# iosefa/obia

Hardware: AMD Instinct MI355X
Metric: Mpixel/s (SLIC+zonal feats) on 16384²×8-band; achieved HBM GB/s fraction (higher is better)
Workload: dtype f32

## Files before the change

### obia_amd/csrc/slic_sweep.hip

```cpp
#include "slic.hpp"

#include <type_traits>
#include <hip/hip_ext.h>

#include <cstdlib>

namespace obia {

#ifdef OBIA_STAMP
__device__ unsigned long long g_tl[65536 * 4 * 24];
#define STAMP_DECL unsigned long long st_t = clock64(), st_t0 = st_t, st_r0 = __builtin_amdgcn_s_memrealtime(), st_acc[12] = {0, 0, 0, 0, 0, 0, 0, 0, 0, 0, 0, 0}, st_cnt[6] = {0, 0, 0, 0, 0, 0};
#define STAMP_COUNT(i, v) st_cnt[i] += (v);
#define STAMP(i) { const unsigned long long st_n = clock64(); st_acc[i] += st_n - st_t; st_t = st_n; }
#ifndef OBIA_STAMP_KIND
#define OBIA_STAMP_KIND 0
#endif
#define STAMP_FLUSH if (accumulate && (LEAN ? 1 : 0) == OBIA_STAMP_KIND && (threadIdx.x & 63) == 0 && gtile < 65536) { unsigned long long *st_o = g_tl + ((size_t)gtile * 4 + (threadIdx.x >> 6)) * 24; for (int st_i = 0; st_i < 12; ++st_i) st_o[st_i] = st_acc[st_i]; st_o[12] = st_t0; st_o[13] = clock64(); st_o[14] = st_r0; st_o[15] = __builtin_amdgcn_s_memrealtime(); for (int st_i = 0; st_i < 6; ++st_i) st_o[16 + st_i] = st_cnt[st_i]; }
#else
#define STAMP_DECL
#define STAMP(i)
#define STAMP_COUNT(i, v)
#define STAMP_FLUSH
#endif

// ... 692 lines not shown
            key = (key == mn) ? 0xffffffffu : key;
            float clb = 0.0f;
            if (COLLB) clb = __uint_as_float(__builtin_amdgcn_readlane(__float_as_uint(clbv), sl));
            const float4 *__restrict__ crec = reinterpret_cast<const float4 *>(cent + (size_t)kk * RS);
            const float4 h0 = crec[0], h1 = crec[1];
            const unsigned mn_next = wave_umin(key);
            const float cy = h0.x, cx = h0.y;
            const int y0 = __float_as_int(h0.z), y1 = __float_as_int(h0.w);
            const int x0 = __float_as_int(h1.x), x1 = __float_as_int(h1.y);
            const float mdc = SLICZERO ? h1.w : 1.0f;
            mn = mn_next;
            STAMP(8)
            const float tx = cx - fx;
            const float dx2 = tx * tx;
            int yb_v = yb_i;
            asm volatile("" : "+v"(yb_v));
            const float fyb = (float)yb_v;
            v2f dv2[PPT / 2];
#pragma unroll
            for (int p = 0; p < PPT / 2; ++p) {
                const v2f tyv = splat(cy) - (splat(fyb) + (v2f){(float)(2 * p), (float)(2 * p + 1)});
                const v2f dy2 = tyv * tyv;
                dv2[p] = (dy2 + splat(dx2)) * splat(w);
            }
            float dv[PPT] = {dv2[0].x, dv2[0].y, dv2[1].x, dv2[1].y};
            if (!((y0 <= fy0) && (y1 >= fy1) && (x0 <= fx0) && (x1 >= fx1))) {
                const bool inx = (x >= x0) && (x < x1);
#pragma unroll
                for (int j = 0; j < PPT; ++j)
                    dv[j] = (inx && ((unsigned)(yb_v + j - y0) < (unsigned)(y1 - y0))) ? dv[j] : INFINITY;
            }
            const bool anylive = COLLB ? (!(dv[0] + clb > BK_D(0)) || !(dv[1] + clb > BK_D(1)) || !(dv[2] + clb > BK_D(2)) || !(dv[3] + clb > BK_D(3)))
                                       : (!(dv[0] > BK_D(0)) || !(dv[1] > BK_D(1)) || !(dv[2] > BK_D(2)) || !(dv[3] > BK_D(3)));
            STAMP_COUNT(1, 1)
            STAMP(9)
            if (!firstv && !__ballot(anylive)) continue;
            STAMP_COUNT(2, 1)
            STAMP_COUNT(3, 2)
            {
                float col[LEAN ? 1 : CP];
                if (!IGNORE_COLOR) {
#pragma unroll
                    for (int q = 0; q < (NCH + 3) / 4; ++q) {
                        const float4 t = crec[2 + q];
                        col[4 * q] = t.x; col[4 * q + 1] = t.y; col[4 * q + 2] = t.z; col[4 * q + 3] = t.w;
                    }
                }
                v2f d0 = (v2f){dv[0], dv[1]}, d1 = (v2f){dv[2], dv[3]};
                if (!IGNORE_COLOR) {
                    v2f t0 = f2[0][0] - splat(col[0]), t1 = f2[0][1] - splat(col[0]);
                    v2f dc0 = t0 * t0, dc1 = t1 * t1;
#pragma unroll
                    for (int ch = 1; ch < (LEAN ? 1 : NCH); ++ch) {
                        t0 = f2[LEAN ? 0 : ch][0] - splat(col[LEAN ? 0 : ch]);
                        t1 = f2[LEAN ? 0 : ch][1] - splat(col[LEAN ? 0 : ch]);
                        dc0 += t0 * t0;
                        dc1 += t1 * t1;
                    }
                    d0 += SLICZERO ? dc0 / splat(mdc) : dc0;
                    d1 += SLICZERO ? dc1 / splat(mdc) : dc1;
                }
                const float dd[PPT] = {d0.x, d0.y, d1.x, d1.y};
                if (firstv) {
#pragma unroll
                    for (int j = 0; j < PPT; ++j) {
                        const unsigned long long nk = ((unsigned long long)__float_as_uint(dd[j]) << 32) | (unsigned long long)c;
                        bk[j] = (dd[j] < INFINITY) ? nk : bk[j];
                    }
                    firstv = false;
                } else
#pragma unroll
                for (int j = 0; j < PPT; ++j) {
                    const unsigned long long nk = ((unsigned long long)__float_as_uint(dd[j]) << 32) | (unsigned long long)c;
                    bk[j] = (nk < bk[j]) ? nk : bk[j];
                }
            }
            mybest = fmaxf(fmaxf(BK_D(0), BK_D(1)), fmaxf(BK_D(2), BK_D(3)));
            STAMP(10)
        }
        STAMP(3)

        int pk[PPT];
        int32_t *lbase = labels + (P.pix_off + (long long)fy0 * P.W + fx0);
        bool orphan = false;
        bool valid[PPT];
#pragma unroll
        for (int j = 0; j < PPT; ++j) {
            const bool inimg = (yb_i + j < P.H) && (x < P.W);
            valid[j] = inimg && (((mbw >> (8 * j)) & 0xffu) != 0u);
            const bool assigned = valid[j] && ((unsigned)(bk[j] >> 32) < INF_BITS);
            pk[j] = assigned ? (int)(unsigned)bk[j] : -1;
            orphan |= valid[j] && !assigned;
        }
        if (store_labels) {
#pragma unroll
            for (int j = 0; j < PPT; ++j) {
                const bool inimg = (yb_i + j < P.H) && (x < P.W);
                const int kk = s_k[(unsigned)bk[j]];
                if (inimg && !(valid[j] && pk[j] < 0))
                    __builtin_nontemporal_store(pk[j] >= 0 ? kk - P.cent_off + start_label : start_label - 1,
                                                lbase + (lrow_i + (unsigned)j * (unsigned)P.W));
            }
        }
        if (__ballot(orphan)) {
            if (orphan_needs_repeat(store_labels, sweep_id) && lane_i == 0) *orphan_flag = 1;
#pragma unroll
            for (int j = 0; j < PPT; ++j)
                if (valid[j] && ((unsigned)(bk[j] >> 32) >= INF_BITS)) {
                    const int ry = yb_i + j - ty0, rx = x - tx0;
                    atomicOr(&s_orph[ry * (SWEEP_TW / 32) + (rx >> 5)], 1u << (rx & 31));
                    s_uncacheable = 1;
                }
        }
        STAMP(4)

        if (accumulate) {
        if (FOLD_LAYERS > 0) s_tkey[wv][0][lane_i] = -1;
        if (FOLD_LAYERS > 1) s_tkey[wv][1][lane_i] = -1;
        {
            const unsigned xrel = (unsigned)(x - tx0);
            int rkey = -1, nruns = 0;
            unsigned pw = 0;
            int rf[LEAN ? 1 : CP];
#pragma unroll
            for (int ch = 0; ch < (LEAN ? 1 : CP); ++ch) rf[ch] = 0;
            auto close_run = [&]() {
                if (rkey < 0) return;
                if (nruns < FOLD_LAYERS) {
                    s_tkey[wv][nruns][lane_i] = rkey;
                    s_tf[wv][nruns][NF - 1][lane_i] = (int)pw;
                    if (!LEAN && accum_color) {
#pragma unroll
                        for (int ch = 0; ch < CP; ++ch) s_tf[wv][nruns][LEAN ? 0 : ch][lane_i] = rf[LEAN ? 0 : ch];
                    }
                } else {
                    atomicAdd(&s_acc[rkey][PWI], (unsigned long long)(pw & 0xffu) | ((unsigned long long)((pw >> 8) & 0xfffu) << 16) |
                                                     ((unsigned long long)(pw >> 20) << 40));
                    if (!LEAN && accum_color) {
#pragma unroll
                        for (int ch = 0; ch < CP; ++ch) atomicAdd(&s_acc[rkey][LEAN ? 0 : ch], (unsigned long long)(long long)rf[LEAN ? 0 : ch]);
                    }
                }
                ++nruns;
            };
            auto merge_strip = [&](auto pre_tag) {
                constexpr bool PRE = decltype(pre_tag)::value;
#pragma unroll
                for (int j = 0; j < PPT; ++j) {
                    if (pk[j] != rkey) {
                        close_run();
                        rkey = pk[j]; pw = 0;
#pragma unroll
                        for (int ch = 0; ch < (LEAN ? 1 : CP); ++ch) rf[ch] = 0;
                    }
                    if (pk[j] >= 0) {
                        pw += 1u | ((unsigned)(yb_i + j - ty0) << 8) | (xrel << 20);
                        if (!LEAN && accum_color) {
#pragma unroll
                            for (int ch = 0; ch < NCH; ++ch) {
                                const float fv = (j & 1) ? f2[LEAN ? 0 : ch][j >> 1].y : f2[LEAN ? 0 : ch][j >> 1].x;
                                rf[LEAN ? 0 : ch] += PRE ? (int)fv : to_fixed32(fv, fs);
                            }
                        }
                    }
                }
                close_run();
            };
            if (fs == 1.0f) merge_strip(std::true_type{});
            else merge_strip(std::false_type{});
        }
        }
        STAMP(5)
        {
            const bool has_next = (bxi + 1 < SWEEP_TW / FB) && (fx0 + FB < P.W);
            fetch(has_next ? fx0 + FB : fx0, yb_i, lane_i, has_next);
        }
        if (!accumulate || FOLD_LAYERS == 0) continue;
        wave_lds_sync();
        if (!LEAN && accum_color) {
#pragma unroll
            for (int pass = 0; pass < NPASS; ++pass) {
                const int fld = 8 * pass + (lane_i & 7), g = lane_i >> 3;
                if (fld < CP) {
#pragma unroll
                    for (int layer = 0; layer < FOLD_LAYERS; ++layer) {
                        int cur = -1;
                        long long sum = 0;
                        int tkv[8], vv[8];
#pragma unroll
                        for (int i = 0; i < 8; ++i) { tkv[i] = s_tkey[wv][layer][8 * g + i]; vv[i] = s_tf[wv][layer][LEAN ? 0 : fld][8 * g + i]; }
#pragma unroll
                        for (int i = 0; i < 8; ++i) {
                            const int tk = tkv[i];
                            const int v = vv[i];
                            if (tk != cur) {
                                if (cur >= 0) atomicAdd(&s_acc[cur][LEAN ? 0 : fld], (unsigned long long)sum);
                                cur = tk; sum = 0;
                            }
                            sum += (long long)v;
                        }
                        if (cur >= 0) atomicAdd(&s_acc[cur][LEAN ? 0 : fld], (unsigned long long)sum);
                    }
                }
            }
        }
        if (lane_i < 8 * FOLD_LAYERS) {
            const int layer = lane_i >> 3, g = lane_i & 7;
            int cur = -1;
            unsigned sum = 0;
            auto emit = [&]() {
                atomicAdd(&s_acc[cur][PWI], (unsigned long long)(sum & 0xffu) | ((unsigned long long)((sum >> 8) & 0xfffu) << 16) |
                                                ((unsigned long long)(sum >> 20) << 40));
            };
            int tkv[8];
            unsigned vv[8];
#pragma unroll
            for (int i = 0; i < 8; ++i) { tkv[i] = s_tkey[wv][layer][8 * g + i]; vv[i] = (unsigned)s_tf[wv][layer][NF - 1][8 * g + i]; }
#pragma unroll
            for (int i = 0; i < 8; ++i) {
                const int tk = tkv[i];
                const unsigned v = vv[i];
                if (tk != cur) {
                    if (cur >= 0) emit();
                    cur = tk; sum = 0;
                }
                sum += v;
            }
            if (cur >= 0) emit();
        }
        wave_lds_sync();
        STAMP(6)
    }
#undef BK_D
    if (!accumulate) { STAMP_FLUSH return; }
    __syncthreads();
    const int tid_e = wv * 64 + lane_now();
    if (s_uncacheable && store_labels == 2) {
        for (int i = tid_e; i < SWEEP_TH * SWEEP_TW; i += NT) {
            if (!((s_orph[i >> 5] >> (i & 31)) & 1u)) continue;
            const int y = ty0 + i / SWEEP_TW, x = tx0 + i % SWEEP_TW;
            const long long pix = P.pix_off + (long long)y * P.W + x;
            const int prev = labels[pix];
            if (prev < start_label) continue;
            float one[CP];
#pragma unroll
            for (int ch = 0; ch < CP; ++ch) one[ch] = (accum_color && ch < nch_rt) ? feat_at(feat, P, CP, y, x, ch) : 0.0f;
            global_accumulate<CP>(acc, RQ, prev - start_label + P.cent_off, (unsigned)y, (unsigned)x, one, fs);
        }
    }
    const bool keep = FIXPT && !s_uncacheable;
    int *ck = keep ? cache_k + (size_t)tile_id * (MAXC + 1) : nullptr;
    unsigned long long *cq = keep ? cache_q + (size_t)tile_id * MAXC * GQ : nullptr;
    constexpr int QLO = (LEAN && !FIXPT) ? CP : 0, QN = GQ - QLO;
    for (int i = tid_e; i < nc * QN; i += NT) {
        const int slot = i / QN, q = QLO + (i - slot * QN);
        const unsigned long long pw = s_acc[slot][PWI];
        const unsigned long long n = pw & 0xffffull;
        if (FIXPT && keep && q == QLO) ck[1 + slot] = n ? s_k[slot] : -1;
        if (n == 0ull) continue;
        const int k = s_k[slot];
        unsigned long long v;
        if (q < CP) { if (!FIXPT && !accum_color) continue; v = accum_color ? s_acc[slot][LEAN ? 0 : q] : 0ull; }
        else if (q == CP) v = n;
        else if (q == CP + 1) v = ((pw >> 16) & 0xffffffull) + n * (unsigned long long)ty0;
        else v = (pw >> 40) + n * (unsigned long long)tx0;
        if (FIXPT && keep) cq[(size_t)slot * GQ + q] = v;
        if (FIXPT && q < CP && !accum_color) continue;
        atomicAdd(&acc[(size_t)k * RQ + q], v);
    }
    if (keep && tid_e == 0) { ck[0] = nc; tile_lp[tile_id] = sweep_id; }
    STAMP(7)
    STAMP_FLUSH
}

#define OBIA_ASSIGN_PARAMS                                                                                             \
    const SlicProblem *__restrict__ probs, const float *__restrict__ feat, const uint8_t *__restrict__ mask,             \
        const unsigned *__restrict__ mask4, const float *__restrict__ cent, const int *__restrict__ head,                                                    \
        int32_t *__restrict__ labels, unsigned long long *__restrict__ acc, int RQ, int accumulate, int store_labels,     \
        int start_label, float fs, const int *__restrict__ bin_stamp, int *__restrict__ tile_lp,                    \
        int *__restrict__ cache_k, unsigned long long *__restrict__ cache_q, int sweep_id, int use_cache,                 \
        unsigned long long *__restrict__ px_counter, const int *__restrict__ tile_prob, int total_tiles_all,              \
        int *__restrict__ orphan_flag, int tiles_per_prob, const float *__restrict__ fbox, int tile_base, int nch_arg,     \
        int *__restrict__ tl_k, unsigned *__restrict__ tl_fp, int *__restrict__ tl_meta, const int *__restrict__ tl_req
#define OBIA_ASSIGN_ARGS                                                                                               \
    probs, feat, mask, mask4, cent, head, labels, acc, RQ, accumulate, store_labels, start_label, fs, bin_stamp, tile_lp, \
        cache_k, cache_q, sweep_id, use_cache, px_counter, tile_prob, total_tiles_all, orphan_flag, tiles_per_prob, fbox, tile_base, nch_arg, \
        tl_k, tl_fp, tl_meta, tl_req

template <int CP, bool MASKED, bool IGNORE_COLOR, bool FIXPT, bool SLICZERO, int NCH = CP>
__global__ __launch_bounds__(NT) __attribute__((amdgpu_waves_per_eu(ASSIGN_WAVES, ASSIGN_WAVES))) void slic_assign_kernel(OBIA_ASSIGN_PARAMS) {
    slic_assign_body<CP, MASKED, IGNORE_COLOR, FIXPT, SLICZERO, false, false, NCH>(OBIA_ASSIGN_ARGS);
}

template <int CP, bool MASKED, int NCH = CP>
__global__ __launch_bounds__(NT) __attribute__((amdgpu_waves_per_eu(6, 6))) void slic_assign_collb_kernel(OBIA_ASSIGN_PARAMS) {
    slic_assign_body<CP, MASKED, false, false, false, false, true, NCH>(OBIA_ASSIGN_ARGS);
}

template <int CP, bool MASKED, bool FIXPT>
__global__ __launch_bounds__(NT) __attribute__((amdgpu_waves_per_eu(LEAN_WAVES, LEAN_WAVES))) void slic_prepass_kernel(OBIA_ASSIGN_PARAMS) {
    slic_assign_body<CP, MASKED, true, FIXPT, false, true, false>(OBIA_ASSIGN_ARGS);
}

#ifdef OBIA_STAMP
extern "C" void obia_debug_timeline(unsigned long long *out, int nwaves) {
    (void)hipMemcpyFromSymbol(out, HIP_SYMBOL(g_tl), sizeof(unsigned long long) * 24 * (size_t)nwaves);
}
#endif

template <int CP, bool MASKED>
__global__ __launch_bounds__(256) void slic_maxdist_kernel(const SlicProblem *__restrict__ probs, const float *__restrict__ feat,
                                                           const uint8_t *__restrict__ mask, const int32_t *__restrict__ labels,
                                                           float *__restrict__ cent, int start_label, int nch) {
    constexpr int RS = CENT_REC + CP;
    const SlicProblem P = probs[blockIdx.y];
    for (int y = blockIdx.x; y < P.H; y += gridDim.x)
        for (int x = threadIdx.x; x < P.W; x += 256) {
            const long long pix = P.pix_off + (long long)y * P.W + x;
            if (MASKED && mask[pix] == 0) continue;
            const int l = labels[pix];
            if (l < start_label) continue;
            const int k = l - start_label + P.cent_off;
            const float *rec = cent + (size_t)k * RS;
            float dc = 0.0f;
#pragma unroll
            for (int ch = 0; ch < CP; ++ch) {
                if (ch >= nch) break;
                const float t = feat_at(feat, P, CP, y, x, ch) - rec[CENT_REC + ch];
                dc += t * t;
            }
            unsigned *slot = reinterpret_cast<unsigned *>(cent + (size_t)k * RS + 7);
            if (__float_as_uint(dc) > __hip_atomic_load(slot, __ATOMIC_RELAXED, __HIP_MEMORY_SCOPE_AGENT)) atomicMax(slot, __float_as_uint(dc));
        }
}

struct FixedPointState {
    int *bin_stamp = nullptr, *tile_lp = nullptr, *cache_k = nullptr;
    unsigned long long *cache_q = nullptr;
};

template <int CP>
static void launch_assign(obia_ctx *ctx, SlicBatch &b, int ignore_color, int accumulate, int accum_color, int store_labels,
                          int *orphan_flag, const FixedPointState &fp, int sweep_id, int use_cache, unsigned long long *px_counter,
                          const KernelSpan &span, const int *head_cur) {
    constexpr int XGH = OBIA_XCD_GROUP;
    const int ntiles = (int)b.total_tiles_all;
    dim3 grid(8 * XGH * (unsigned)((ntiles + 8 * XGH - 1) / (8 * XGH)));
    const int RQ = acc_record_qwords(CP);
    int tpp = b.probs.empty() ? 0 : b.probs[0].tiles_x * b.probs[0].tiles_y;
    for (auto &P : b.probs) if (P.tiles_x * P.tiles_y != tpp) tpp = 0;
#define LAUNCH_K_(...)                                                                                               \
    hipExtLaunchKernelGGL(HIP_KERNEL_NAME(__VA_ARGS__), grid, dim3(NT), 0, ctx->stream, span.a, span.b, 0, b.d_probs, b.d_feat,   \
                          b.d_mask, b.d_mask4, b.d_cent, head_cur, b.d_labels, b.d_acc, RQ, accumulate, store_labels, b.start_label,      \
                          (float)b.fscale, fp.bin_stamp, fp.tile_lp, fp.cache_k, fp.cache_q, sweep_id, use_cache, px_counter,          \
                          b.d_tile_prob, ntiles, orphan_flag, tpp, b.d_fbox, 0, b.C, b.d_tl_k, b.d_tl_fp, b.d_tl_meta, b.d_tl_req)
    const int pad = CP - b.C;
#define LAUNCH_ASSIGN_(M, I, F, Z) LAUNCH_K_(slic_assign_kernel<CP, M, I, F, Z>)
#define LAUNCH_MAIN_(M)                                                                                              \
    do {                                                                                                             \
        if (pad == 1) LAUNCH_K_(slic_assign_kernel<CP, M, false, false, false, CP - 1>);                             \
        else if (pad == 2) LAUNCH_K_(slic_assign_kernel<CP, M, false, false, false, CP - 2>);                        \
        else if (pad == 3) LAUNCH_K_(slic_assign_kernel<CP, M, false, false, false, CP - 3>);                        \
        else LAUNCH_K_(slic_assign_kernel<CP, M, false, false, false>);                                              \
    } while (0)
#define LAUNCH_COLLB_(M)                                                                                             \
    do {                                                                                                             \
        if (pad == 1) LAUNCH_K_(slic_assign_collb_kernel<CP, M, CP - 1>);                                            \
        else if (pad == 2) LAUNCH_K_(slic_assign_collb_kernel<CP, M, CP - 2>);                                       \
        else if (pad == 3) LAUNCH_K_(slic_assign_collb_kernel<CP, M, CP - 3>);                                       \
        else LAUNCH_K_(slic_assign_collb_kernel<CP, M>);                                                             \
    } while (0)
#define LAUNCH_LEAN_(M, F) LAUNCH_K_(slic_prepass_kernel<CP, M, F>)
#define LAUNCH_ASSIGN(M, I)                                                                                          \
    do {                                                                                                             \
        if ((I) && !accum_color) { if (fp.bin_stamp) LAUNCH_LEAN_(M, true); else LAUNCH_LEAN_(M, false); }           \
        else if (b.slic_zero && !(I)) LAUNCH_ASSIGN_(M, false, false, true);                                         \
        else if (fp.bin_stamp) LAUNCH_ASSIGN_(M, I, true, false);                                                    \
        else if (b.col_lb && b.d_fbox && !(I)) LAUNCH_COLLB_(M);                                                     \
        else if (!(I)) LAUNCH_MAIN_(M);                                                                              \
        else LAUNCH_ASSIGN_(M, I, false, false);                                                                     \
    } while (0)
    if (b.masked) { if (ignore_color) LAUNCH_ASSIGN(true, true); else LAUNCH_ASSIGN(true, false); }
    else LAUNCH_ASSIGN(false, false);
#undef LAUNCH_ASSIGN
#undef LAUNCH_ASSIGN_
#undef LAUNCH_LEAN_
#undef LAUNCH_COLLB_
#undef LAUNCH_MAIN_
#undef LAUNCH_K_
}

__global__ __launch_bounds__(256) void mask_pack4_kernel(const SlicProblem *__restrict__ probs, const uint8_t *__restrict__ mask,
                                                         unsigned *__restrict__ mask4) {
    const SlicProblem P = probs[blockIdx.y];
    if ((long long)P.n_valid == (long long)P.H * (long long)P.W) return;
    const int nq = (P.H + 3) >> 2, W = P.W;
    const uint8_t *mb = mask + P.pix_off;
    unsigned *out = mask4 + P.m4_off;
    const bool vec = (W % 4 == 0) && (P.pix_off % 4 == 0) && (P.m4_off % 4 == 0) && (reinterpret_cast<uintptr_t>(mask) % 4 == 0) &&
                     (reinterpret_cast<uintptr_t>(mask4) % 16 == 0);
    for (int q = blockIdx.x; q < nq; q += gridDim.x) {
        if (vec) {
            for (int x4 = threadIdx.x; x4 < (W >> 2); x4 += 256) {
                unsigned r[4];
#pragma unroll
                for (int j = 0; j < 4; ++j) {
                    const int y = 4 * q + j;
                    r[j] = y < P.H ? *reinterpret_cast<const unsigned *>(mb + (long long)y * W + 4 * x4) : 0u;
                }
                uint4 o;
                unsigned *ov = &o.x;
#pragma unroll
                for (int c = 0; c < 4; ++c) {
                    unsigned w = 0u;
#pragma unroll
                    for (int j = 0; j < 4; ++j) w |= (unsigned)(((r[j] >> (8 * c)) & 0xffu) != 0u) << (8 * j);
                    ov[c] = w;
                }
                *reinterpret_cast<uint4 *>(out + (long long)q * W + 4 * x4) = o;
            }
        } else {
            for (int x = threadIdx.x; x < W; x += 256) {
                unsigned w = 0u;
#pragma unroll
                for (int j = 0; j < 4; ++j) {
                    const int y = 4 * q + j;
                    if (y < P.H) w |= (unsigned)(mb[(long long)y * W + x] != 0) << (8 * j);
                }
                out[(long long)q * W + x] = w;
            }
        }
    }
}

__global__ void fill_i32_kernel(int32_t *p, long long n, int32_t v) {
    for (long long i = (long long)blockIdx.x * blockDim.x + threadIdx.x; i < n; i += (long long)gridDim.x * blockDim.x) p[i] = v;
}

static void fill_labels(obia_ctx *ctx, SlicBatch &b) {
    const long long n = b.total_pix;
    int blocks = cdiv(n, 256 * 8);
    if (blocks > 65535) blocks = 65535;
    if (blocks < 1) blocks = 1;
    hipLaunchKernelGGL(fill_i32_kernel, dim3(blocks), dim3(256), 0, ctx->stream, b.d_labels, n, b.start_label - 1);
}

static void fold_counters(obia_ctx *ctx, const unsigned long long *h) {
    if (ctx->profiling)
        for (int i = 0; i < 256; ++i) { ctx->timing.assign_px += (double)h[i]; ctx->timing.prepass_px += (double)h[256 + i]; }
}

static int queue_sweeps(obia_ctx *ctx, SlicBatch &b, bool repeat, unsigned long long **d_px_out) {
    *d_px_out = nullptr;
    if (std::getenv("OBIA_DEBUG_SYNC"))
        for (size_t p = 0; p < b.probs.size(); ++p) {
            const SlicProblem &P = b.probs[p];
            fprintf(stderr, "[obia debug]   problem %zu: %dx%d K %d steps %d %d bins %dx%d cell_off %d cent_off %d tiles %dx%d tile_off %d n_valid %d (total_cent %d total_cells %d tiles_all %lld)\n",
                    p, P.H, P.W, P.K, P.sy, P.sx, P.ncy, P.ncx, P.cell_off, P.cent_off, P.tiles_y, P.tiles_x, P.tile_off, P.n_valid,
                    b.total_cent, b.total_cells, b.total_tiles_all);
        }
    if (b.total_tiles <= 0 || b.max_iter <= 0) { fill_labels(ctx, b); return OBIA_OK; }
    for (auto &P : b.probs)
        if (P.W >= (1 << 22)) { set_error("rasters / tile windows wider than 4194303 pixels are not supported (got %d)", P.W); return OBIA_E_UNSUPPORTED; }
    const int passes = b.masked ? 2 : 1;
    const int RQ = acc_record_qwords(b.CP);
    Arena &A = ctx->arena;
    unsigned long long *d_px = A.get<unsigned long long>(513);
    if (!d_px) return OBIA_E_NOMEM;
    int *d_orphan = reinterpret_cast<int *>(d_px + 512);
    FixedPointState fp;
    if (b.exit_on_fixed_point) {
        const size_t nt = (size_t)b.total_tiles_all;
        fp.bin_stamp = A.get<int>((size_t)b.total_cells);
        fp.tile_lp = A.get<int>(nt);
        fp.cache_k = A.get<int>(nt * (MAXC + 1));
        fp.cache_q = A.get<unsigned long long>(nt * MAXC * (size_t)(b.CP + 3));
        if (!fp.bin_stamp || !fp.tile_lp || !fp.cache_k || !fp.cache_q) return OBIA_E_NOMEM;
        OBIA_HIP_TRY(hipMemsetAsync(fp.bin_stamp, 0, sizeof(int) * (size_t)b.total_cells, ctx->stream));
        OBIA_HIP_TRY(hipMemsetAsync(fp.tile_lp, 0, sizeof(int) * nt, ctx->stream));
    }
    {
        const size_t nt = (size_t)b.total_tiles_all;
        b.d_tl_k = A.get<int>(nt * MAXC);
        b.d_tl_fp = A.get<unsigned>(nt * NT);
        b.d_tl_meta = A.get<int>(nt * 3);
        b.d_tl_req = b.d_tl_meta ? b.d_tl_meta + nt * 2 : nullptr;
        b.d_ref = A.get<float>((size_t)b.total_cent * 2);
        if (!b.d_tl_k || !b.d_tl_fp || !b.d_tl_meta || !b.d_tl_req || !b.d_ref) return OBIA_E_NOMEM;
    }
    int maxh_z = 1, kmax = 1;
    for (auto &P : b.probs) { if (P.H > maxh_z) maxh_z = P.H; if (P.K > kmax) kmax = P.K; }
    if (b.masked && b.d_mask && !b.d_mask4) {
        b.d_mask4 = A.get<unsigned>((size_t)b.total_m4);
        if (!b.d_mask4) return OBIA_E_NOMEM;
        int gq = (maxh_z + 3) / 4;
        if (gq > 16384) gq = 16384;
        hipLaunchKernelGGL(mask_pack4_kernel, dim3(gq, b.nprob), dim3(256), 0, ctx->stream, b.d_probs, b.d_mask, b.d_mask4);
    }
    if (maxh_z > 4096) maxh_z = 4096;

    const bool store_all = repeat || b.exit_on_fixed_point || b.slic_zero;
    if (store_all || passes * b.max_iter <= 1) {
        fill_labels(ctx, b);
        debug_sync(ctx, "sweeps: label fill");
    }
    if (repeat) OBIA_HIP_TRY(hipMemsetAsync(b.d_acc, 0, sizeof(unsigned long long) * (size_t)b.total_cent * RQ, ctx->stream));
    const bool prep_grouped = std::getenv("OBIA_PREP_GROUPED") != nullptr;
    OBIA_HIP_TRY(hipMemsetAsync(d_px, 0, sizeof(unsigned long long) * 513, ctx->stream));
    OBIA_HIP_TRY(hipMemsetAsync(b.d_head, 0xff, sizeof(int) * (size_t)b.total_cells, ctx->stream));
    OBIA_HIP_TRY(hipMemsetAsync(b.d_tl_meta, 0xff, sizeof(int) * 3 * (size_t)b.total_tiles_all, ctx->stream));
    debug_sync(ctx, "sweeps: memsets");
    bool first = true;
    int sweep_no = 0;
    for (int pass = 0; pass < passes; ++pass) {
        const int ignore_color = (b.masked && pass == 0) ? 1 : 0;
        const bool last_pass = (pass == passes - 1);
        if (pass > 0 && store_all) {
            fill_labels(ctx, b);
            if (fp.tile_lp) OBIA_HIP_TRY(hipMemsetAsync(fp.tile_lp, 0, sizeof(int) * (size_t)b.total_tiles_all, ctx->stream));
        }
        for (int it = 0; it < b.max_iter; ++it) {
            int *head_cur = b.d_head + (size_t)(sweep_no & 1) * b.total_cells;
            int *head_nxt = b.d_head + (size_t)((sweep_no + 1) & 1) * b.total_cells;
            ++sweep_no;
            const int zmode = (b.slic_zero && !ignore_color) ? (it == 0 ? 2 : 1) : 0;
#define LAUNCH_PREP_LANE(CPV)                                                                                         \
    hipLaunchKernelGGL(HIP_KERNEL_NAME(slic_prep_lane_kernel<CPV>), dim3(cdiv(kmax, 64), b.nprob), dim3(64), 0, ctx->stream, \
                       b.d_probs, 0, first ? 1 : 0, zmode, b.d_seed, b.d_acc, RQ, 1.0 / b.fscale, b.d_cent, head_cur, head_nxt, \
                       b.total_cells, fp.bin_stamp, sweep_no, 0, b.d_ref, b.d_tl_req)
            if (!prep_grouped) {
                switch (b.CP) {
                    case 4: LAUNCH_PREP_LANE(4); break;
                    case 8: LAUNCH_PREP_LANE(8); break;
                    case 12: LAUNCH_PREP_LANE(12); break;
                    default: LAUNCH_PREP_LANE(16); break;
                }
            } else if (RQ == 16)
                hipLaunchKernelGGL(HIP_KERNEL_NAME(slic_prep_kernel<16>), dim3(cdiv(b.total_cent * 16LL, 256)), dim3(256), 0,
                                   ctx->stream, b.d_probs, b.d_cent_prob, b.total_cent, b.CP, first ? 1 : 0, zmode, b.d_seed, b.d_acc,
                                   1.0 / b.fscale, b.d_cent, head_cur, head_nxt, b.total_cells, fp.bin_stamp, sweep_no, 0, 0, b.d_ref, b.d_tl_req);
            else
                hipLaunchKernelGGL(HIP_KERNEL_NAME(slic_prep_kernel<32>), dim3(cdiv(b.total_cent * 32LL, 256)), dim3(256), 0,
                                   ctx->stream, b.d_probs, b.d_cent_prob, b.total_cent, b.CP, first ? 1 : 0, zmode, b.d_seed, b.d_acc,
                                   1.0 / b.fscale, b.d_cent, head_cur, head_nxt, b.total_cells, fp.bin_stamp, sweep_no, 0, 0, b.d_ref, b.d_tl_req);
#undef LAUNCH_PREP_LANE
            b.d_head_cur = head_cur;
            debug_sync(ctx, "sweeps: prep");
            first = false;
            if (zmode == 1) {
                dim3 zg(maxh_z, b.nprob);
#define LAUNCH_MAXDIST(CPV)                                                                                           \
    do {                                                                                                              \
        if (b.masked) hipLaunchKernelGGL(HIP_KERNEL_NAME(slic_maxdist_kernel<CPV, true>), zg, dim3(256), 0, ctx->stream, b.d_probs, \
                                         b.d_feat, b.d_mask, b.d_labels, b.d_cent, b.start_label, b.C);            \
        else hipLaunchKernelGGL(HIP_KERNEL_NAME(slic_maxdist_kernel<CPV, false>), zg, dim3(256), 0, ctx->stream, b.d_probs, \
                                b.d_feat, b.d_mask, b.d_labels, b.d_cent, b.start_label, b.C);                     \
    } while (0)
                switch (b.CP) {
                    case 4: LAUNCH_MAXDIST(4); break;
                    case 8: LAUNCH_MAXDIST(8); break;
                    case 12: LAUNCH_MAXDIST(12); break;
                    default: LAUNCH_MAXDIST(16); break;
                }
#undef LAUNCH_MAXDIST
            }
            const bool very_last = last_pass && it == b.max_iter - 1;
            const int accumulate = very_last ? 0 : 1;
            const int accum_color = (!ignore_color || it == b.max_iter - 1) ? 1 : 0;
            const int store_labels = store_all ? 2 : (very_last ? 1 : 0);
            const int use_cache = (ignore_color && it == b.max_iter - 1) ? 0 : 1;
            {
                KernelSpan span(ctx, ignore_color ? T_PREPASS : T_ASSIGN);
                unsigned long long *pxc = ctx->profiling ? d_px + (ignore_color ? 256 : 0) : nullptr;
                if (ctx->profiling && !ignore_color && store_labels) ctx->timing.assign_store_px += (double)b.total_pix;
                switch (b.CP) {
                    case 8: launch_assign<8>(ctx, b, ignore_color, accumulate, accum_color, store_labels, d_orphan, fp, sweep_no, use_cache, pxc, span, head_cur); break;
#ifndef OBIA_ONLY_CP8
                    case 4: launch_assign<4>(ctx, b, ignore_color, accumulate, accum_color, store_labels, d_orphan, fp, sweep_no, use_cache, pxc, span, head_cur); break;
                    case 12: launch_assign<12>(ctx, b, ignore_color, accumulate, accum_color, store_labels, d_orphan, fp, sweep_no, use_cache, pxc, span, head_cur); break;
                    case 16: launch_assign<16>(ctx, b, ignore_color, accumulate, accum_color, store_labels, d_orphan, fp, sweep_no, use_cache, pxc, span, head_cur); break;
#endif
                    default: set_error("bad CP"); return OBIA_E_INVALID;
                }
            }
            debug_sync(ctx, ignore_color ? "sweeps: pre-pass sweep" : "sweeps: colour sweep");
        }
    }
    OBIA_HIP_TRY(hipGetLastError());
    *d_px_out = d_px;
    return OBIA_OK;
}

int slic_run_sweeps(obia_ctx *ctx, SlicBatch &b) {
    ctx->defer_pending = false;
    unsigned long long *d_px = nullptr;
    OBIA_TRY(queue_sweeps(ctx, b, false, &d_px));
    if (!d_px) return OBIA_OK;
    if (!ctx->defer_buf) OBIA_HIP_TRY(hipHostMalloc(reinterpret_cast<void **>(&ctx->defer_buf), sizeof(unsigned long long) * 513, hipHostMallocDefault));
    OBIA_HIP_TRY(hipMemcpyAsync(ctx->defer_buf, d_px, sizeof(unsigned long long) * 513, hipMemcpyDeviceToHost, ctx->stream));
    ctx->defer_pending = true;
    return OBIA_OK;
}

int slic_sweeps_settle(obia_ctx *ctx, bool *repeat) {
    *repeat = false;
    if (!ctx->defer_pending) return OBIA_OK;
    ctx->defer_pending = false;
    const unsigned long long *h = ctx->defer_buf;
    if ((h[512] & 0xffffffffull) != 0ull) { *repeat = true; return OBIA_OK; }
    fold_counters(ctx, h);
    return OBIA_OK;
}

int slic_rerun_storing(obia_ctx *ctx, SlicBatch &b) {
    ctx->timing.batch_repeats += 1;
    unsigned long long *d_px = nullptr;
    OBIA_TRY(queue_sweeps(ctx, b, true, &d_px));
    if (!d_px) return OBIA_OK;
    unsigned long long h[513];
    OBIA_TRY(read_back(ctx, h, d_px, sizeof(h)));
    fold_counters(ctx, h);
    return OBIA_OK;
}

}
```

Before: 6489.

## Add run-based spatial-only prepass kernel exploiting distance convexity along rows

Adds a specialized kernel for the spatial-only (ignore-colour) prepass sweeps. Each 16-pixel row run is assigned by evaluating candidate centroids only at its endpoints (plus a split point), and falls back to per-pixel queues when margins are too small. Candidates are pruned per 16x16 block with lower and upper distance bounds, and counts and coordinate sums are accumulated as packed LDS atomics. This replaces per-pixel distance evaluation in masked prepass sweeps that do not store labels, at the cost of added code complexity and floating-point tie-margin heuristics.

```diff
diff --git a/obia_amd/csrc/slic_spatial.hip b/obia_amd/csrc/slic_spatial.hip
--- /dev/null
+++ b/obia_amd/csrc/slic_spatial.hip
@@ -0,0 +1,284 @@
+
+#ifdef OBIA_RUN_STATS
+__device__ unsigned long long g_run_stats[16];
+#define RS_DECL unsigned long long rs_t = clock64(); unsigned rs_c[8] = {0, 0, 0, 0, 0, 0, 0, 0};
+#define RS_COUNT(i, v) rs_c[i] += (unsigned)(v);
+#define RS_TICK(i) { const unsigned long long rs_n = clock64(); if ((threadIdx.x & 63) == 0) atomicAdd(&g_run_stats[i], rs_n - rs_t); rs_t = rs_n; }
+#define RS_FLUSH { for (int rs_i = 1; rs_i < 8; ++rs_i) { unsigned rs_v = rs_c[rs_i]; for (int rs_o = 32; rs_o; rs_o >>= 1) rs_v += __shfl_xor(rs_v, rs_o); \
+                   if ((threadIdx.x & 63) == 0) atomicAdd(&g_run_stats[rs_i], (unsigned long long)rs_v); } if ((threadIdx.x & 63) == 0) atomicAdd(&g_run_stats[0], 1ull); }
+extern "C" void obia_debug_run_stats(unsigned long long *out, int reset) {
+    (void)hipMemcpyFromSymbol(out, HIP_SYMBOL(g_run_stats), sizeof(unsigned long long) * 16);
+    if (reset) { unsigned long long z[16] = {0}; (void)hipMemcpyToSymbol(HIP_SYMBOL(g_run_stats), z, sizeof(z)); }
+}
+#else
+#define RS_DECL
+#define RS_COUNT(i, v)
+#define RS_TICK(i)
+#define RS_FLUSH
+#endif
+
+constexpr float RUN_REL = 0x1p-19f, RUN_ABS = 0x1p-60f, RUN_W_LO = 0x1p-30f, RUN_W_HI = 0x1p90f;
+
+template <int CP>
+__device__ __forceinline__ void slic_spatial_tile(const SlicProblem &P, int gtile, int tile, int l_n, const unsigned *__restrict__ mask4,
+                                                  const float *__restrict__ cent, unsigned long long *__restrict__ acc, int RQ,
+                                                  unsigned long long *__restrict__ px_counter, int *__restrict__ orphan_flag,
+                                                  const int *__restrict__ tl_k, const unsigned *__restrict__ tl_fp) {
+    constexpr int RS = CENT_REC + CP;
+    constexpr int NW = NT / 64;
+    constexpr unsigned INF_BITS = 0x7f800000u;
+    __shared__ __attribute__((aligned(16))) float r_hdr[MAXC][CENT_REC];
+    __shared__ int r_k[MAXC];
+    __shared__ unsigned long long r_acc[MAXC];
+    __shared__ unsigned char r_surv[NW][SWEEP_TW / FB][64];
+    __shared__ unsigned r_q[NW][128];
+
+    const int tid = threadIdx.x;
+    const int wv = __builtin_amdgcn_readfirstlane(tid >> 6);
+    const int ty0 = (tile / P.tiles_x) * SWEEP_TH, tx0 = (tile % P.tiles_x) * SWEEP_TW;
+    const float w = P.spatial_w;
+    RS_DECL
+    if (px_counter && tile == 0 && tid == 0) atomicAdd(px_counter, (unsigned long long)P.H * (unsigned long long)P.W);
+
+    int lk = -1;
+    if (tid < l_n) lk = tl_k[(size_t)gtile * MAXC + tid];
+    const unsigned myc4 = tl_fp[(size_t)gtile * NT + tid];
+    if (tid < MAXC) r_acc[tid] = 0ull;
+    if (lk >= 0) {
+        const float4 *src = reinterpret_cast<const float4 *>(cent + (size_t)lk * RS);
+        const float4 a = src[0], b = src[1];
+        float4 *dh = reinterpret_cast<float4 *>(&r_hdr[tid][0]);
+        dh[0] = a; dh[1] = b;
+        r_k[tid] = lk;
+    }
+    const int nc = l_n;
+    __syncthreads();
+    RS_TICK(8)
+
+    const int fy0 = ty0 + FB * wv;
+    if (fy0 < P.H) {
+        const int fy1 = min(fy0 + FB, P.H);
+        const int lane = lane_now();
+        int cnt[SWEEP_TW / FB];
+#pragma unroll
+        for (int bxi = 0; bxi < SWEEP_TW / FB; ++bxi) {
+            const int fx0 = tx0 + FB * bxi;
+            cnt[bxi] = 0;
+            if (fx0 >= P.W) continue;
+            const int fx1 = min(fx0 + FB, P.W);
+            const unsigned c = (myc4 >> (8 * bxi)) & 0xffu;
+            unsigned lbb = 0xffffffffu, ubb = INF_BITS;
+            bool hit = false;
+            if (c != 0xffu) {
+                const float4 h0 = *reinterpret_cast<const float4 *>(&r_hdr[c][0]);
+                const float2 h1 = *reinterpret_cast<const float2 *>(&r_hdr[c][4]);
+                const int y0 = __float_as_int(h0.z), y1 = __float_as_int(h0.w), x0 = __float_as_int(h1.x), x1 = __float_as_int(h1.y);
+                if (y0 < fy1 && y1 > fy0 && x0 < fx1 && x1 > fx0) {
+                    hit = true;
+                    const float cy = h0.x, cx = h0.y;
+                    const float ylo = (float)fy0, yhi = (float)(fy1 - 1), xlo = (float)fx0, xhi = (float)(fx1 - 1);
+                    const float ry = (cy < ylo) ? ylo : ((cy > yhi) ? yhi : cy), rx = (cx < xlo) ? xlo : ((cx > xhi) ? xhi : cx);
+                    const float tyn = cy - ry, txn = cx - rx;
+                    lbb = __float_as_uint((tyn * tyn + txn * txn) * w);
+                    if (y0 <= fy0 && y1 >= fy1 && x0 <= fx0 && x1 >= fx1) {
+                        const float tyf = fmaxf(fabsf(cy - ylo), fabsf(cy - yhi)), txf = fmaxf(fabsf(cx - xlo), fabsf(cx - xhi));
+                        ubb = __float_as_uint((tyf * tyf + txf * txf) * w);
+                    }
+                }
+            }
+            const unsigned bound = wave_umin(ubb);
+            bool surv = hit && lbb <= bound;
+            if (bound != INF_BITS) {
+                const int la = (int)__builtin_ctzll(__ballot(ubb == bound));
+                const int ca = __builtin_amdgcn_readlane((int)c, la);
+                const float4 ha = *reinterpret_cast<const float4 *>(&r_hdr[ca][0]);
+                const float4 hb = *reinterpret_cast<const float4 *>(&r_hdr[surv ? c : ca][0]);
+                const float ylo = (float)fy0, yhi = (float)(fy1 - 1), xlo = (float)fx0, xhi = (float)(fx1 - 1);
+                const float ay0 = (ha.x - ylo) * (ha.x - ylo), ay1 = (ha.x - yhi) * (ha.x - yhi), ax0 = (ha.y - xlo) * (ha.y - xlo), ax1 = (ha.y - xhi) * (ha.y - xhi);
+                const float by0 = (hb.x - ylo) * (hb.x - ylo), by1 = (hb.x - yhi) * (hb.x - yhi), bx0 = (hb.y - xlo) * (hb.y - xlo), bx1 = (hb.y - xhi) * (hb.y - xhi);
+                const float a00 = (ay0 + ax0) * w, a01 = (ay0 + ax1) * w, a10 = (ay1 + ax0) * w, a11 = (ay1 + ax1) * w;
+                const float g = fminf(fminf((by0 + bx0) * w - a00, (by0 + bx1) * w - a01), fminf((by1 + bx0) * w - a10, (by1 + bx1) * w - a11));
+                const float M = fmaxf(fmaxf(a00, a01), fmaxf(a10, a11));
+                if (M < 3.0e38f && g > RUN_REL * M + RUN_ABS * w) surv = false;
+            }
+            const unsigned long long m = __ballot(surv);
+            const unsigned pos = __builtin_amdgcn_mbcnt_hi((unsigned)(m >> 32), __builtin_amdgcn_mbcnt_lo((unsigned)m, 0u));
+            if (surv) r_surv[wv][bxi][pos] = (unsigned char)c;
+            cnt[bxi] = __popcll(m);
+        }
+        wave_lds_sync();
+        RS_TICK(9)
+
+        const int seg = lane >> 4, y = fy0 + (lane & 15), xa = tx0 + FB * seg;
+        const int mycnt = seg == 0 ? cnt[0] : (seg == 1 ? cnt[1] : (seg == 2 ? cnt[2] : cnt[3]));
+        const unsigned char *sv = &r_surv[wv][seg][0];
+        unsigned rowbits = 0u;
+        if (y < P.H && xa < P.W) {
+            const int n = min(FB, P.W - xa);
+            if ((long long)P.n_valid == (long long)P.H * (long long)P.W) {
+                rowbits = 0xffffu >> (FB - n);
+            } else {
+                const unsigned *mp = mask4 + ((long long)P.m4_off + (long long)(y >> 2) * P.W + xa);
+                const int sh = 8 * (y & 3);
+#pragma unroll
+                for (int i = 0; i < FB; ++i) {
+                    const unsigned v = (i < n) ? mp[i] : 0u;
+                    rowbits |= (unsigned)(((v >> sh) & 0xffu) != 0u) << i;
+                }
+            }
+        }
+        const float fy = (float)y;
+        bool orphan = false;
+        auto add_run = [&](int k, int a, int b) {
+            const unsigned bits = rowbits & (0xffffu >> (FB - 1 - (b - xa))) & (0xffffu << (a - xa)) & 0xffffu;
+            if (!bits) return;
+            if (k < 0) { orphan = true; return; }
+            const unsigned m = __popc(bits);
+            const unsigned sx = __popc(bits & 0xaaaau) + 2u * __popc(bits & 0xccccu) + 4u * __popc(bits & 0xf0f0u) + 8u * __popc(bits & 0xff00u) +
+                                m * (unsigned)(xa - tx0);
+            RS_COUNT(7, 1)
+            atomicAdd(&r_acc[k], (unsigned long long)m | ((unsigned long long)(m * (unsigned)(y - ty0)) << 16) | ((unsigned long long)sx << 40));
+        };
+        auto take = [](float d, bool in, int c, float &d1, float &d2, int &k1) {
+            const bool t = in && d < d1;
+            d2 = fminf(d2, t ? d1 : d);
+            d1 = t ? d : d1;
+            k1 = t ? c : k1;
+        };
+        const float abs_w = RUN_ABS * w;
+        auto margin = [&](float d1a, float d2a, float d1b, float d2b) {
+            const float M = fmaxf(d1a, d1b);
+            return M < 3.0e38f && fminf(d2a - d1a, d2b - d1b) > RUN_REL * M + abs_w;
+        };
+        auto entry = [&](int a, int b) {
+            return (unsigned)(a - xa) | ((unsigned)(b - xa) << 4) | ((unsigned)(lane & 15) << 8) | ((unsigned)seg << 12) | (rowbits << 16);
+        };
+        unsigned q0 = 0xffffffffu, q1 = 0xffffffffu;
+        if (rowbits) {
+            const int xl = xa + __builtin_ctz(rowbits), xr = xa + 31 - __builtin_clz(rowbits);
+            const float fxl = (float)xl, fxr = (float)xr;
+            float d1l = INFINITY, d2l = INFINITY, d1r = INFINITY, d2r = INFINITY;
+            int k1l = -1, k1r = -1;
+            for (int i = 0; i < mycnt; ++i) {
+                const int c = sv[i];
+                const float4 h0 = *reinterpret_cast<const float4 *>(&r_hdr[c][0]);
+                const float2 h1 = *reinterpret_cast<const float2 *>(&r_hdr[c][4]);
+                const int y0 = __float_as_int(h0.z), y1 = __float_as_int(h0.w), x0 = __float_as_int(h1.x), x1 = __float_as_int(h1.y);
+                if ((unsigned)(y - y0) >= (unsigned)(y1 - y0)) continue;
+                const float ty = h0.x - fy, dy2 = ty * ty;
+                const float tl = h0.y - fxl, tr = h0.y - fxr;
+                take((dy2 + tl * tl) * w, xl >= x0 && xl < x1, c, d1l, d2l, k1l);
+                take((dy2 + tr * tr) * w, xr >= x0 && xr < x1, c, d1r, d2r, k1r);
+            }
+            const int len = xr - xl + 1;
+            RS_COUNT(1, 1) RS_COUNT(2, mycnt)
+            if (k1l >= 0 && k1l == k1r && (len == 1 || margin(d1l, d2l, d1r, d2r))) {
+                RS_COUNT(3, 1)
+                add_run(k1l, xl, xr);
+            } else if (len <= 2) {
+                add_run(k1l, xl, xl);
+                if (len == 2) add_run(k1r, xr, xr);
+            } else if (len >= 4 && k1l >= 0 && k1r >= 0 && k1l != k1r) {
+                RS_COUNT(4, 1)
+                const float4 ha = *reinterpret_cast<const float4 *>(&r_hdr[k1l][0]), hb = *reinterpret_cast<const float4 *>(&r_hdr[k1r][0]);
+                const float tya = ha.x - fy, tyb = hb.x - fy, txa = ha.y - fxr, txb = hb.y - fxl;
+                const float gl = (tyb * tyb + txb * txb) * w - d1l, gr = (tya * tya + txa * txa) * w - d1r;
+                int m = xl + (int)(gl / (gl + gr) * (float)(len - 1));
+                m = max(xl + 1, min(m, xr - 2));
+                const int p0 = m - 1, p3 = m + 2;
+                const float fp0 = (float)p0, fm = (float)m, fm1 = (float)(m + 1), fp3 = (float)p3;
+                float e1p0 = INFINITY, e2p0 = INFINITY, e1p3 = INFINITY, e2p3 = INFINITY, e1m = INFINITY, e1m1 = INFINITY, dump = INFINITY;
+                int kp0 = -1, kp3 = -1, km = -1, km1 = -1;
+                for (int i = 0; i < mycnt; ++i) {
+                    const int c = sv[i];
+                    const float4 h0 = *reinterpret_cast<const float4 *>(&r_hdr[c][0]);
+                    const float2 h1 = *reinterpret_cast<const float2 *>(&r_hdr[c][4]);
+                    const int y0 = __float_as_int(h0.z), y1 = __float_as_int(h0.w), x0 = __float_as_int(h1.x), x1 = __float_as_int(h1.y);
+                    if ((unsigned)(y - y0) >= (unsigned)(y1 - y0)) continue;
+                    const float ty = h0.x - fy, dy2 = ty * ty;
+                    const float t0 = h0.y - fp0, t1 = h0.y - fm, t2 = h0.y - fm1, t3 = h0.y - fp3;
+                    take((dy2 + t0 * t0) * w, p0 >= x0 && p0 < x1, c, e1p0, e2p0, kp0);
+                    take((dy2 + t1 * t1) * w, m >= x0 && m < x1, c, e1m, dump, km);
+                    take((dy2 + t2 * t2) * w, m + 1 >= x0 && m + 1 < x1, c, e1m1, dump, km1);
+                    take((dy2 + t3 * t3) * w, p3 >= x0 && p3 < x1, c, e1p3, e2p3, kp3);
+                }
+                const bool okl = kp0 == k1l && (p0 == xl || margin(d1l, d2l, e1p0, e2p0));
+                const bool okr = kp3 == k1r && (p3 == xr || margin(e1p3, e2p3, d1r, d2r));
+                bool mdone = false, m1done = false;
+                if (okl) { mdone = km == k1l; add_run(k1l, xl, mdone ? m : p0); } else q0 = entry(xl, p0);
+                if (okr) { m1done = km1 == k1r; add_run(k1r, m1done ? m + 1 : p3, xr); } else q1 = entry(p3, xr);
+                if (!mdone) add_run(km, m, m);
+                if (!m1done) add_run(km1, m + 1, m + 1);
+            } else {
+                q0 = entry(xl, xr);
+            }
+        }
+        int qn = 0;
+        {
+            const unsigned long long m0 = __ballot(q0 != 0xffffffffu);
+            if (q0 != 0xffffffffu) r_q[wv][__builtin_amdgcn_mbcnt_hi((unsigned)(m0 >> 32), __builtin_amdgcn_mbcnt_lo((unsigned)m0, 0u))] = q0;
+            qn = __popcll(m0);
+            const unsigned long long m1 = __ballot(q1 != 0xffffffffu);
+            if (q1 != 0xffffffffu) r_q[wv][qn + __builtin_amdgcn_mbcnt_hi((unsigned)(m1 >> 32), __builtin_amdgcn_mbcnt_lo((unsigned)m1, 0u))] = q1;
+            qn += __popcll(m1);
+        }
+        wave_lds_sync();
+        RS_TICK(10)
+        RS_COUNT(5, lane == 0 ? qn : 0)
+        for (int base = 0; base < qn; base += 4) {
+            const int ei = base + (lane >> 4);
+            if (ei >= qn) continue;
+            const unsigned e = r_q[wv][ei];
+            const int xrel = (int)(e & 15u) + (lane & 15);
+            if (xrel > (int)((e >> 4) & 15u) || !((e >> (16 + xrel)) & 1u)) continue;
+            RS_COUNT(6, 1)
+            const int qs = (int)((e >> 12) & 3u), qy = fy0 + (int)((e >> 8) & 15u), qx = tx0 + FB * qs + xrel;
+            const int qcnt = qs == 0 ? cnt[0] : (qs == 1 ? cnt[1] : (qs == 2 ? cnt[2] : cnt[3]));
+            const unsigned char *qv = &r_surv[wv][qs][0];
+            const float fqy = (float)qy, fqx = (float)qx;
+            float best = INFINITY;
+            int bk = -1;
+            for (int i = 0; i < qcnt; ++i) {
+                const int c = qv[i];
+                const float4 h0 = *reinterpret_cast<const float4 *>(&r_hdr[c][0]);
+                const float2 h1 = *reinterpret_cast<const float2 *>(&r_hdr[c][4]);
+                const int y0 = __float_as_int(h0.z), y1 = __float_as_int(h0.w), x0 = __float_as_int(h1.x), x1 = __float_as_int(h1.y);
+                if (!(qy >= y0 && qy < y1 && qx >= x0 && qx < x1)) continue;
+                const float ty = h0.x - fqy, tx = h0.y - fqx;
+                const float d = (ty * ty + tx * tx) * w;
+                if (d < best) { best = d; bk = c; }
+            }
+            if (bk < 0) orphan = true;
+            else atomicAdd(&r_acc[bk], 1ull | ((unsigned long long)(unsigned)(qy - ty0) << 16) | ((unsigned long long)(unsigned)(qx - tx0) << 40));
+        }
+        if (__ballot(orphan) && lane == 0) *orphan_flag = 1;
+        RS_TICK(11)
+        RS_FLUSH
+    }
+    __syncthreads();
+    const int tid_e = wv * 64 + lane_now();
+    for (int i = tid_e; i < nc * 3; i += NT) {
+        const int slot = i / 3, q = i - slot * 3;
+        const unsigned long long pw = r_acc[slot];
+        const unsigned long long n = pw & 0xffffull;
+        if (n == 0ull) continue;
+        const unsigned long long v = q == 0 ? n : (q == 1 ? ((pw >> 16) & 0xffffffull) + n * (unsigned long long)ty0 : (pw >> 40) + n * (unsigned long long)tx0);
+        atomicAdd(&acc[(size_t)r_k[slot] * RQ + CP + q], v);
+    }
+    RS_TICK(12)
+}
+
+template <int CP>
+__global__ __launch_bounds__(NT) __attribute__((amdgpu_waves_per_eu(LEAN_WAVES, LEAN_WAVES))) void slic_spatial_kernel(OBIA_ASSIGN_PARAMS) {
+    constexpr int XG = OBIA_XCD_GROUP;
+    const int gtile = tile_base + (((int)(blockIdx.x >> 3) / XG) * 8 + (int)(blockIdx.x & 7)) * XG + (int)(blockIdx.x >> 3) % XG;
+    if (gtile >= total_tiles_all) return;
+    const int l_n = tl_meta[2 * (size_t)gtile], l_bw = tl_meta[2 * (size_t)gtile + 1], l_req = tl_req[gtile];
+    const int prob_i = tiles_per_prob > 0 ? gtile / tiles_per_prob : tile_prob[gtile];
+    const SlicProblem P = probs[prob_i];
+    const bool listed = l_n >= 0 && l_bw >= 0 && l_req <= (l_bw & 0xffff);
+    if (listed && accumulate && !store_labels && !P.direct && P.spatial_w >= RUN_W_LO && P.spatial_w <= RUN_W_HI)
+        slic_spatial_tile<CP>(P, gtile, gtile - P.tile_off, l_n, mask4, cent, acc, RQ, px_counter, orphan_flag, tl_k, tl_fp);
+    else
+        slic_assign_body<CP, true, true, false, false, true, false>(OBIA_ASSIGN_ARGS);
+}
diff --git a/obia_amd/csrc/slic_sweep.hip b/obia_amd/csrc/slic_sweep.hip
--- a/obia_amd/csrc/slic_sweep.hip
+++ b/obia_amd/csrc/slic_sweep.hip
@@ -1018,6 +1018,8 @@
     slic_assign_body<CP, MASKED, true, FIXPT, false, true, false>(OBIA_ASSIGN_ARGS);
 }
 
+#include "slic_spatial.hip"
+
 #ifdef OBIA_STAMP
 extern "C" void obia_debug_timeline(unsigned long long *out, int nwaves) {
     (void)hipMemcpyFromSymbol(out, HIP_SYMBOL(g_tl), sizeof(unsigned long long) * 24 * (size_t)nwaves);
@@ -1058,7 +1060,7 @@
 template <int CP>
 static void launch_assign(obia_ctx *ctx, SlicBatch &b, int ignore_color, int accumulate, int accum_color, int store_labels,
                           int *orphan_flag, const FixedPointState &fp, int sweep_id, int use_cache, unsigned long long *px_counter,
-                          const KernelSpan &span, const int *head_cur) {
+                          const KernelSpan &span, const int *head_cur, bool prepass_visits) {
     constexpr int XGH = OBIA_XCD_GROUP;
     const int ntiles = (int)b.total_tiles_all;
     dim3 grid(8 * XGH * (unsigned)((ntiles + 8 * XGH - 1) / (8 * XGH)));
@@ -1089,7 +1091,11 @@
 #define LAUNCH_LEAN_(M, F) LAUNCH_K_(slic_prepass_kernel<CP, M, F>)
 #define LAUNCH_ASSIGN(M, I)                                                                                          \
     do {                                                                                                             \
-        if ((I) && !accum_color) { if (fp.bin_stamp) LAUNCH_LEAN_(M, true); else LAUNCH_LEAN_(M, false); }           \
+        if ((I) && !accum_color) {                                                                                   \
+            if (fp.bin_stamp) LAUNCH_LEAN_(M, true);                                                                 \
+            else if (store_labels || prepass_visits) LAUNCH_LEAN_(M, false);                                         \
+            else LAUNCH_K_(slic_spatial_kernel<CP>);                                                                 \
+        }                                                                                                            \
         else if (b.slic_zero && !(I)) LAUNCH_ASSIGN_(M, false, false, true);                                         \
         else if (fp.bin_stamp) LAUNCH_ASSIGN_(M, I, true, false);                                                    \
         else if (b.col_lb && b.d_fbox && !(I)) LAUNCH_COLLB_(M);                                                     \
@@ -1222,6 +1228,7 @@
     }
     if (repeat) OBIA_HIP_TRY(hipMemsetAsync(b.d_acc, 0, sizeof(unsigned long long) * (size_t)b.total_cent * RQ, ctx->stream));
     const bool prep_grouped = std::getenv("OBIA_PREP_GROUPED") != nullptr;
+    const bool prepass_visits = std::getenv("OBIA_PREPASS_VISITS") != nullptr;
     OBIA_HIP_TRY(hipMemsetAsync(d_px, 0, sizeof(unsigned long long) * 513, ctx->stream));
     OBIA_HIP_TRY(hipMemsetAsync(b.d_head, 0xff, sizeof(int) * (size_t)b.total_cells, ctx->stream));
     OBIA_HIP_TRY(hipMemsetAsync(b.d_tl_meta, 0xff, sizeof(int) * 3 * (size_t)b.total_tiles_all, ctx->stream));
@@ -1290,11 +1297,11 @@
                 unsigned long long *pxc = ctx->profiling ? d_px + (ignore_color ? 256 : 0) : nullptr;
                 if (ctx->profiling && !ignore_color && store_labels) ctx->timing.assign_store_px += (double)b.total_pix;
                 switch (b.CP) {
-                    case 8: launch_assign<8>(ctx, b, ignore_color, accumulate, accum_color, store_labels, d_orphan, fp, sweep_no, use_cache, pxc, span, head_cur); break;
+                    case 8: launch_assign<8>(ctx, b, ignore_color, accumulate, accum_color, store_labels, d_orphan, fp, sweep_no, use_cache, pxc, span, head_cur, prepass_visits); break;
 #ifndef OBIA_ONLY_CP8
-                    case 4: launch_assign<4>(ctx, b, ignore_color, accumulate, accum_color, store_labels, d_orphan, fp, sweep_no, use_cache, pxc, span, head_cur); break;
-                    case 12: launch_assign<12>(ctx, b, ignore_color, accumulate, accum_color, store_labels, d_orphan, fp, sweep_no, use_cache, pxc, span, head_cur); break;
-                    case 16: launch_assign<16>(ctx, b, ignore_color, accumulate, accum_color, store_labels, d_orphan, fp, sweep_no, use_cache, pxc, span, head_cur); break;
+                    case 4: launch_assign<4>(ctx, b, ignore_color, accumulate, accum_color, store_labels, d_orphan, fp, sweep_no, use_cache, pxc, span, head_cur, prepass_visits); break;
+                    case 12: launch_assign<12>(ctx, b, ignore_color, accumulate, accum_color, store_labels, d_orphan, fp, sweep_no, use_cache, pxc, span, head_cur, prepass_visits); break;
+                    case 16: launch_assign<16>(ctx, b, ignore_color, accumulate, accum_color, store_labels, d_orphan, fp, sweep_no, use_cache, pxc, span, head_cur, prepass_visits); break;
 #endif
                     default: set_error("bad CP"); return OBIA_E_INVALID;
                 }
```

New measurement: 6744 (median of 6 runs). 3.9% higher.
